# VIS4ROB-lab/ccm_slam

Hardware: AMD Instinct MI355X
Metric: global-BA LM iterations/s (4-agent merged map) (higher is better)
Workload: dtype f64; 1 GPU; gba_c4: global BA (MapFusionGBA numerics), 2000 KFs / 150000 landmarks / 954782 observations, Huber sqrt(5.99), landmark-sharded x1

## Files before the change

### ccm_slam_amd/csrc/ba.hip

```cpp
#include "common.h"
#include "test_internal.h"
#include "ba_types.h"
#include "lane_xor.h"
#include "ba_math.h"
#include <algorithm>
#include <chrono>
#include <cmath>
#include <cstring>
#include <limits>
#include <numeric>

int ccm_allreduce_f64(ccm_ctx* ctx, double* d_buf, size_t n);
int ccm_allreduce_max_f64(ccm_ctx* ctx, double* d_buf, size_t n);

namespace {


inline double now_ms() {
  return std::chrono::duration<double, std::milli>(std::chrono::steady_clock::now().time_since_epoch()).count();
}

__device__ __forceinline__ double wave_sum(double v) { return lanex::wave_sum(v); }

__device__ __forceinline__ double block_sum(double v, double* lds ) {
// ... 1035 lines not shown
    }
    asm volatile("s_waitcnt lgkmcnt(0)" ::: "memory");
  }
  if (el) {
#pragma unroll
    for (int pq = 0; pq < 4; pq++) part[wv][pq][lane] = acc[pq];
  }
  __syncthreads();
  if (threadIdx.x < 4 * 36) {
    const int pq = threadIdx.x / 36, e = threadIdx.x % 36;
    double tot = 0;
#pragma unroll
    for (int k = 0; k < kNW; k++) tot += part[k][pq][e];
    stage_out[((size_t)w * 4 + pq) * 36 + e] = tot;
  }
}

__global__ void ba_coarse_sum(const double* stage, const unsigned* cb_key, int n_cb, int na, int nn, double* Ac, int Nc) {
  const size_t idx = (size_t)blockIdx.x * blockDim.x + threadIdx.x;
  if (idx >= (size_t)Nc * Nc) return;
  const int row = (int)(idx / Nc), col = (int)(idx % Nc);
  if (row >= 6 * nn || col >= 6 * nn) { Ac[idx] = (row == col) ? 1.0 : 0.0; return; }
  int n = row / 6, r = row % 6, n2 = col / 6, c = col % 6;
  if (row > col) { int tmp = n; n = n2; n2 = tmp; tmp = r; r = c; c = tmp; }
  double sum = 0;
#pragma unroll
  for (int pq = 0; pq < 4; pq++) {
    const int p = pq >> 1, q = pq & 1;
    int a = n - p, b = n2 - q;
    if (a < 0 || b < 0 || a >= na || b >= na) continue;
    int sel = 2 * p + q, e = r * 6 + c;
    if (a > b) { const int tmp = a; a = b; b = tmp; sel = 2 * q + p; e = c * 6 + r; }
    const unsigned key = (unsigned)a * (unsigned)na + (unsigned)b;
    int lo = 0, hi = n_cb;
    while (lo < hi) { const int mid = (lo + hi) >> 1; if (cb_key[mid] < key) lo = mid + 1; else hi = mid; }
    if (lo < n_cb && cb_key[lo] == key) sum += stage[((size_t)lo * 4 + sel) * 36 + e];
  }
  Ac[idx] = sum;
}

constexpr long kPersMaxSpins = 8000;
constexpr int kPersCooldownTrials = 8;

struct PersArgs {
  double lambda, rel_tol;
  int max_it, n_clu;
  unsigned* bar;
  int test_abort;
  const int* coff; const int* cij; const uint32_t* cblk;
  unsigned long long* slots;
  unsigned long long* utag;
  unsigned long long* tag;
  int prefetch;
  unsigned long long epoch_base;
  const int* uoff;
  const int* ucol;
  const int* loc;
  long long* dbg;
  const double* Ainv; const double* Pm; int na, Nc;
  double* wsave; int w_load;
};

__device__ __forceinline__ double pers_uniform(double v) {
  const long long b = __double_as_longlong(v);
  const int lo = __builtin_amdgcn_readfirstlane((int)(b & 0xffffffffll)), hi = __builtin_amdgcn_readfirstlane((int)(b >> 32));
  return __longlong_as_double(((long long)hi << 32) | (unsigned int)lo);
}

typedef unsigned int pers_u32x4 __attribute__((ext_vector_type(4)));
constexpr int kAuxSc1 = 16;
__device__ __forceinline__ void tag_store(__amdgpu_buffer_rsrc_t rs, unsigned byte_off, double v, unsigned long long key) {
  const unsigned long long b = (unsigned long long)__double_as_longlong(v), c = b ^ key;
  pers_u32x4 q;
  q.x = (unsigned)b; q.y = (unsigned)(b >> 32); q.z = (unsigned)c; q.w = (unsigned)(c >> 32);
  __builtin_amdgcn_raw_buffer_store_b128(q, rs, (int)byte_off, 0, kAuxSc1);
}
__device__ __forceinline__ pers_u32x4 tag_load(__amdgpu_buffer_rsrc_t rs, unsigned byte_off) { return __builtin_amdgcn_raw_buffer_load_b128(rs, (int)byte_off, 0, kAuxSc1); }
__device__ __forceinline__ bool tag_valid(pers_u32x4 q, unsigned long long key) {
  return (q.x ^ q.z) == (unsigned)key && (q.y ^ q.w) == (unsigned)(key >> 32);
}
__device__ __forceinline__ double tag_value(pers_u32x4 q) { return __longlong_as_double((long long)(((unsigned long long)q.y << 32) | q.x)); }

template <class Mid>
__device__ __forceinline__ bool pers_exchange(int t , unsigned long long* slots , int nwg, int me, double a_thread, double b_thread,
                                              bool force_nan, unsigned long long epoch, unsigned* abort_flag, double* red ,
                                              double* total_a, double* total_b, int* poll_fail ,
                                              Mid&& mid ) {
  const unsigned long long key = 0x9E3779B97F4A7C15ull * epoch;
  {
    const double wa = wave_sum(a_thread), wb = wave_sum(b_thread);
    if ((t & (kWave - 1)) == 0) { red[t / kWave] = wa; red[kPersWaves + t / kWave] = wb; }
  }
  __syncthreads();
  if (t == 0) {
    double ma = 0, mb = 0;
#pragma unroll
    for (int w = 0; w < kPersWaves; w++) { ma += red[w]; mb += red[kPersWaves + w]; }
    if (force_nan) ma = __longlong_as_double(0x7ff8000000000000ll);
    const unsigned long long ba = (unsigned long long)__double_as_longlong(ma), bb = (unsigned long long)__double_as_longlong(mb);
    __hip_atomic_store(slots + me, ba, __ATOMIC_RELAXED, __HIP_MEMORY_SCOPE_AGENT);
    __hip_atomic_store(slots + nwg + me, bb, __ATOMIC_RELAXED, __HIP_MEMORY_SCOPE_AGENT);
    __hip_atomic_store(slots + 2 * nwg + me, ba ^ bb ^ key, __ATOMIC_RELAXED, __HIP_MEMORY_SCOPE_AGENT);
  }
  if (t < kWave) {
    constexpr int kPer = 4;
    unsigned done = 0;
    double va[kPer], vb[kPer];
#pragma unroll
    for (int j = 0; j < kPer; j++) { va[j] = 0; vb[j] = 0; if (t + j * kWave >= nwg) done |= 1u << j; }
    bool ok_w = true;
    for (long spins = 0;; spins++) {
#pragma unroll
      for (int j = 0; j < kPer; j++) {
        if (done & (1u << j)) continue;
        const unsigned long long* in = slots + t + j * kWave;
        const unsigned long long b0 = __hip_atomic_load(in, __ATOMIC_RELAXED, __HIP_MEMORY_SCOPE_AGENT);
        const unsigned long long b1 = __hip_atomic_load(in + nwg, __ATOMIC_RELAXED, __HIP_MEMORY_SCOPE_AGENT);
        const unsigned long long b2 = __hip_atomic_load(in + 2 * nwg, __ATOMIC_RELAXED, __HIP_MEMORY_SCOPE_AGENT);
        if ((b0 ^ b1 ^ b2) == key) { done |= 1u << j; va[j] = __longlong_as_double((long long)b0); vb[j] = __longlong_as_double((long long)b1); }
      }
      if (__all(done == (1u << kPer) - 1u)) break;
      if (spins > kPersMaxSpins || __hip_atomic_load(abort_flag, __ATOMIC_RELAXED, __HIP_MEMORY_SCOPE_AGENT) != 0u) { ok_w = false; break; }
      __builtin_amdgcn_s_sleep(2);
    }
    const double sa = wave_sum(((va[0] + va[1]) + va[2]) + va[3]);
    const double sb = wave_sum(((vb[0] + vb[1]) + vb[2]) + vb[3]);
    if (t == 0) {
      red[2 * kPersWaves] = sa; red[2 * kPersWaves + 1] = sb;
      if (!ok_w) { *poll_fail = 1; __hip_atomic_store(abort_flag, 1u, __ATOMIC_RELAXED, __HIP_MEMORY_SCOPE_AGENT); }
    }
  } else {
    mid();
  }
  __syncthreads();
  const bool alive = *poll_fail == 0;
  *total_a = pers_uniform(red[2 * kPersWaves]);
  *total_b = pers_uniform(red[2 * kPersWaves + 1]);
  return alive;
}

#define PERS_TICK(slot) { if (timing) { const long long tn_ = wall_clock64(); tacc[slot] += tn_ - tacc[12]; tacc[12] = tn_; } }

__device__ __forceinline__ double pers_bcast(double v, int src_lane) {
  const long long b = __double_as_longlong(v);
  const int lo = __builtin_amdgcn_readlane((int)(b & 0xffffffffll), src_lane), hi = __builtin_amdgcn_readlane((int)(b >> 32), src_lane);
  double r = __longlong_as_double(((long long)hi << 32) | (unsigned int)lo);
  asm volatile("" : "+v"(r));
  return r;
}

__device__ __noinline__ void pers_assemble_cluster(double* A, double* Li, const int* cij, const uint32_t* cblk, int c_lo, int c_hi, const double* S, int m,
                                                   double lambda, bool has) {
  constexpr int N = kCluN;
  const int t = threadIdx.x;
  for (int i = t; i < N * N; i += kPersTPB) { A[i] = 0; Li[i] = 0; }
  __syncthreads();
  if (has) {
    const int grp = t / 36, e = t % 36, r = e / 6, cc = e % 6;
    constexpr int kGroups = kPersTPB / 36;
    if (grp < kGroups)
#pragma unroll 4
      for (int s = c_lo + grp; s < c_hi; s += kGroups) {
        const int ij = cij[s], il = ij >> 4, jl = ij & 15;
        const uint32_t bt = cblk[s];
        const double* B = S + 36 * (size_t)(bt & ~kTransposeBit);
        const double v = (bt & kTransposeBit) ? B[cc * 6 + r] : B[e];
        A[(6 * il + r) * N + 6 * jl + cc] = v + ((il == jl && r == cc) ? lambda : 0.0);
      }
  }
  if (m + t < N) A[(m + t) * N + m + t] = 1.0;
  __syncthreads();
}

__device__ __noinline__ void pers_factor_dense(double* A, double* Li, int* ibuf, int m, long long* tacc, bool timing) {
  constexpr int N = kCluN;
  const int t = threadIdx.x;
  PERS_TICK(7)
  double* invd = Li;
  {
    typedef double v4d __attribute__((ext_vector_type(4)));
    const int lane = t & (kWave - 1), wave = __builtin_amdgcn_readfirstlane(t / kWave);
    const int i16 = lane & 15, kq = lane >> 4;
    for (int T = 0; T < 6 && 16 * T < m; T++) {
      const int b0 = 16 * T;
      const int r0 = b0 + 16;
      if (wave < 2) {
        const int rl = lane & 15;
        const int prow = r0 + 48 * wave + (lane - 16);
        const bool is_panel = lane >= 16;
        const int rowi = is_panel ? min(prow, N - 1) : b0 + rl;
        double row[16];
#pragma unroll
        for (int k = 0; k < 16; k++) row[k] = A[rowi * N + b0 + k];
        bool bad = false;
#pragma unroll
        for (int c = 0; c < 16; c++) {
          double sv = row[c];
#pragma unroll
          for (int k = 0; k < c; k++) sv = fma(-row[k], pers_bcast(row[k], c), sv);
          double dd = pers_bcast(sv, c);
          if (!(dd > 0.0)) { bad = true; dd = 1.0; }
          const double inv = rsqrt(dd);
// ... 525 lines not shown
        if (t == c) xres = xc;
      }
      xv[16 * I + t] = xres;
    }
    __syncthreads();
#pragma unroll
    for (int s = 0; s < kCRSlots; s++) {
      const int ij = CR_TIJ(s);
      if ((ij >> 8) == I && (ij & 255) < I) {
        const int J = ij & 255;
        double pv = 0.0;
#pragma unroll
        for (int r = 0; r < 4; r++) pv = fma(acc[s][r], xv[16 * I + kq + 4 * r], pv);
        pv = lanex::add_partner<16>(pv);
        pv = lanex::add_partner<32>(pv);
        if (kq == 0) yv[16 * J + i16] -= pv;
      }
    }
    __syncthreads();
  }
  if (t < n) d.x[t] = xv[t];
  CR_TICK(2)
  {
    double sc = 0;
    if (t < Cp) {
      const int c = d.slot_cam[t];
      double u[6];
#pragma unroll
      for (int q = 0; q < 6; q++) u[q] = xv[6 * t + q];
      const BaPose Tc = ba_load_pose(d.cam[cur] + 7 * (size_t)c);
      const BaPose Tn = ba_oplus(u, Tc);
      ba_store_pose(d.cam[cur ^ 1] + 7 * (size_t)c, Tn);
#pragma unroll
      for (int q = 0; q < 6; q++) sc += u[q] * ((add_lambda_term ? lambda * u[q] : 0.0) + d.bp[6 * (size_t)t + q]);
    }
    if (t < kWave) {
      const double s = wave_sum(sc);
      if (t == 0) d.part_cam[0] = ((s + 0.0) + 0.0) + 0.0;
    }
  }
  CR_TICK(3)
  if (dbg && t == 0) dbg[7] += 1;
#undef CR_TICK
#undef CR_TIJ
  if (t == 0) { d.pcg_flag[0] = 1; d.pcg_flag[1] = 1; d.pcg_flag[2] = ibuf[1]; d.pcg_flag[3] = 0; }
}

__global__ __launch_bounds__(kPersTPB) void ba_pcg_persist(BaDev d, PersArgs a) {
  extern __shared__ __attribute__((aligned(16))) double sm[];
  constexpr int N = kCluN;
  double* A = sm;
  double* Li = sm + N * N;
  double* rc = Li + N * N;
  double* xs = rc + N;
  double* ps = xs + N / 2;
  double* ss = ps + N / 2;
  double* zs = ss + N;
  double* zpart = zs + N;
  double* wl = zpart + 4 * N;
  double* pso = zpart + 8 * N;
  double* red = pso + kPersNcCap;
  int* ibuf = reinterpret_cast<int*>(red + 2 * kPersWaves + 4);
  if (a.test_abort && blockIdx.x == gridDim.x - 1) return;
  const int t = threadIdx.x, lane = t & (kWave - 1);
  const int wv = __builtin_amdgcn_readfirstlane(t / kWave);
  const int nwg = gridDim.x;
  const int per_xcd = nwg >> 3;
  const int u = (blockIdx.x & 7) * per_xcd + (blockIdx.x >> 3);
  const int c = u >> 1, hu = u & 1;
  const bool has = c < a.n_clu;
  const int s0 = has ? c * kClu : 0, s1 = has ? min(d.Cp, s0 + kClu) : 0;
  const int nrows = s1 - s0;
  const int m = 6 * nrows;
  const int o0 = has ? min(s1, s0 + (kClu / 2) * hu) : 0, o1 = has ? min(s1, o0 + kClu / 2) : 0;
  const int nown = o1 - o0;
  const int mo = 6 * nown;
  const int ob = 6 * (o0 - s0);
  unsigned long long epoch = a.epoch_base;
  const double lambda = a.lambda;
  if (t < 4) ibuf[t] = (t == 0) ? 1 : 0;
  long long* tacc = reinterpret_cast<long long*>(ibuf + 4);
  const bool timing = a.dbg != nullptr && blockIdx.x == 0 && t == 0;
  if (timing) { for (int q = 0; q < 12; q++) tacc[q] = 0; tacc[12] = wall_clock64(); }
  if (a.w_load) {
    const double* src = a.wsave + (size_t)u * (N * (N / 2));
    double wreg[5];
    int nw = 0;
    for (int e = t; e < N * (N / 2); e += kPersTPB, nw++) wreg[nw] = src[e];
    nw = 0;
    for (int e = t; e < N * (N / 2); e += kPersTPB, nw++) A[e] = wreg[nw];
    __syncthreads();
  } else {
    pers_factor_cluster(A, Li, ibuf, a.cij, a.cblk, has ? a.coff[c] : 0, has ? a.coff[c + 1] : 0, d.S, s0, s1, lambda, has, tacc, timing);
    double wreg[5];
    int nw = 0;
    for (int e = t; e < N * (N / 2); e += kPersTPB, nw++) wreg[nw] = A[(e / (N / 2)) * N + ob + e % (N / 2)];
    __syncthreads();
    nw = 0;
    double* dst = a.wsave ? a.wsave + (size_t)u * (N * (N / 2)) : nullptr;
    for (int e = t; e < N * (N / 2); e += kPersTPB, nw++) { A[e] = wreg[nw]; if (dst) dst[e] = wreg[nw]; }
  }
  const bool coarse = a.Ainv != nullptr;
  const int Nc = a.Nc, nca = 6 * (a.na + 1);
  float* ainv_l = reinterpret_cast<float*>(A + N * (N / 2));
  double* rco = Li + (32 + 2 * kPersIdxCap + kPersColCap) / 2 + 6 * kPersColCap + 256;
  double* pown = rco + Nc;
  double* ypart = pown + 8 * 36;
  constexpr int kParkA = 8 * N - (4 * N + N / 2);
  double* park_a = zpart + 4 * N + N / 2;
  double* park_b = ypart + 12;
  auto park = [&](int x) { return x < kParkA ? park_a + x : park_b + (x - kParkA); };
  static_assert((32 + 2 * kPersIdxCap + kPersColCap) % 2 == 0 &&
                (32 + 2 * kPersIdxCap + kPersColCap) / 2 + 6 * kPersColCap + 256 + kPersNcCap + 8 * 36 + 12 + (N + kPersNcCap - kParkA) <= kCluN * kCluN,
                "coarse vectors and the parked values do not fit behind the staged structure");
  const int aggu = d.agg >> 3;
  const int agg = u / aggu;
  if (coarse) {
    {
      const double* src = a.Ainv + (size_t)(6 * agg) * Nc;
      double tmpa[9];
#pragma unroll
      for (int q = 0; q < 9; q++) { const int e = t + q * kPersTPB; tmpa[q] = (has && e < 12 * Nc) ? src[e] : 0.0; }
#pragma unroll
      for (int q = 0; q < 9; q++) { const int e = t + q * kPersTPB; if (e < 12 * Nc) ainv_l[e] = (float)tmpa[q]; }
    }
    for (int e = t; e < Nc; e += kPersTPB) { rco[e] = 0.0; pso[e] = 0.0; }
    for (int e = t; e < 8 * 36; e += kPersTPB) pown[e] = (e / 36 < nown) ? a.Pm[36 * (size_t)o0 + e] : 0.0;
  }
  __syncthreads();
  int tq = t, lq = lane;
  auto key_of = [](unsigned long long e) { return 0x9E3779B97F4A7C15ull * e; };
  const unsigned tag_w_pairs = 2u * 6u * (unsigned)d.Cp;
  const __amdgpu_buffer_rsrc_t tag_rs = __builtin_amdgcn_make_buffer_rsrc(a.tag, 0, (int)(16u * (tag_w_pairs + 2u * 8u * (unsigned)kPersNcCap)), 0x00020000);
  auto w_off = [&](unsigned long long e, int i) { return 16u * ((unsigned)(e & 1) * 6u * (unsigned)d.Cp + (unsigned)i); };
  auto c_off = [&](unsigned long long e, int pl, int j) { return 16u * (tag_w_pairs + ((unsigned)(e & 1) * 8u + (unsigned)pl) * (unsigned)kPersNcCap + (unsigned)j); };
  auto coarse_restrict = [&](const double* vec , unsigned long long e ) {
    if (wv == 0) {
      const int cc = lq >> 3, kk = lq & 7;
      double sv = 0;
      if (cc < 6 && kk < nown) {
#pragma unroll
        for (int rr = 0; rr < 6; rr++) sv += pown[kk * 36 + rr * 6 + cc] * vec[6 * kk + rr];
      }
      const double w1 = coarse_hat_t(8 * u + kk, d.agg);
      double s0v = (1.0 - w1) * sv, s1v = w1 * sv;
      s0v = lanex::add_partner<1>(s0v); s1v = lanex::add_partner<1>(s1v);
      s0v = lanex::add_partner<2>(s0v); s1v = lanex::add_partner<2>(s1v);
      s0v = lanex::add_partner<4>(s0v); s1v = lanex::add_partner<4>(s1v);
      if (cc < 6 && kk == 0 && agg < a.na) { tag_store(tag_rs, c_off(e, u - aggu * agg, 6 * agg + cc), s0v, key_of(e)); tag_store(tag_rs, c_off(e, 4 + u - aggu * agg, 6 * (agg + 1) + cc), s1v, key_of(e)); }
    }
  };
  auto fetch_pre = [&](unsigned long long e, bool want_w) {
    const unsigned long long key = key_of(e);
    int tf = tq;
    asm volatile("" : "+v"(tf));
    const int p = tf - kWave, j = p - N;
    const bool is_w = want_w && p >= 0 && p < m && !(p >= ob && p < ob + mo);
    const bool is_c = coarse && j >= 0 && j < nca;
    const int n = j / 6;
    bool ok = true;
    double sgm = 0;
    for (int h = 0; h < 2 && 2 * h < aggu; h++) {
      unsigned off[2] = {c_off(e, 2 * h, j), c_off(e, 4 + 2 * h, j)}, want = 0;
#pragma unroll
      for (int i = 0; i < 4; i++) {
        const int mm = 2 * h + (i >> 1);
        const bool first = (i & 1) == 0;
        const int unit = first ? aggu * n + mm : aggu * (n - 1) + mm;
        if (is_c && mm < aggu && (first ? n < a.na : n >= 1) && unit < nwg) want |= 1u << i;
      }
      if (is_w) { want = (h == 0) ? 1u : 0u; off[0] = w_off(e, 6 * s0 + p); }
      unsigned todo = want;
      pers_u32x4 q[4];
#pragma unroll
      for (int i = 0; i < 4; i++) q[i] = pers_u32x4{0u, 0u, 0u, 0u};
      for (int spins = 0; todo; spins++) {
        asm volatile("" ::: "memory");
#pragma unroll
        for (int i = 0; i < 4; i++) if (todo & (1u << i)) q[i] = tag_load(tag_rs, off[i & 1] + 16u * (unsigned)kPersNcCap * (unsigned)(i >> 1));
#pragma unroll
        for (int i = 0; i < 4; i++) if ((todo & (1u << i)) && tag_valid(q[i], key)) todo &= ~(1u << i);
        if (!todo) break;
        if (spins > kPersMaxSpins || __hip_atomic_load(a.bar + 1, __ATOMIC_RELAXED, __HIP_MEMORY_SCOPE_AGENT) != 0u) { ok = false; break; }
        __builtin_amdgcn_s_sleep(1);
      }
      if (is_w) { if (h == 0) *park(p) = tag_value(q[0]); }
      else {
#pragma unroll
        for (int i = 0; i < 4; i++) if (want & (1u << i)) sgm += tag_value(q[i]);
      }
      if (!ok) break;
    }
    if (is_c) *park(p) = sgm;
    if (!ok) { ibuf[2] = 1; __hip_atomic_store(a.bar + 1, 1u, __ATOMIC_RELAXED, __HIP_MEMORY_SCOPE_AGENT); }
  };
  if (t < N / 2) { xs[t] = 0; ps[t] = 0; }
  if (t < N) { ss[t] = 0; zs[t] = 0; rc[t] = (t < m) ? d.bs[6 * (size_t)s0 + t] : 0.0; }
  __syncthreads();
  PERS_TICK(10)
  int* l_off = reinterpret_cast<int*>(Li);
  int* l_loc = l_off + 32;
  uint32_t* l_blk = reinterpret_cast<uint32_t*>(l_loc + kPersIdxCap);
  int* l_ucol = reinterpret_cast<int*>(l_blk + kPersIdxCap);
  double* pl = reinterpret_cast<double*>(l_ucol + kPersColCap);
  double* half_sum = pl + 6 * kPersColCap;
  const int e_base = has ? d.row_off[o0] : 0;
  const int n_ent = has ? d.row_off[o1] - e_base : 0;
  const int u_base = has ? a.uoff[u] : 0;
  const int nu = has ? a.uoff[u + 1] - u_base : 0;
  if (has) {
    if (t <= nown) l_off[t] = d.row_off[o0 + t] - e_base;
    for (int s = t; s < n_ent; s += kPersTPB) { l_loc[s] = a.loc[e_base + s]; l_blk[s] = d.row_blk[e_base + s]; }
    for (int s = t; s < nu; s += kPersTPB) l_ucol[s] = a.ucol[u_base + s];
  }
  if (t < 6) pl[t] = 0.0;
  __syncthreads();
  constexpr int kPersRegEnt = 5;
  const int row_l = wv >> 1, half = wv & 1, g = lane / 6, r = lane % 6;
  const bool row_ok = has && row_l < nown && g < 10;
  double sreg[kPersRegEnt][6];
  int jreg[kPersRegEnt];
  {
    const int e0 = row_ok ? l_off[row_l] : 0;
    const int e_end = row_ok ? l_off[row_l + 1] : 0;
#pragma unroll
    for (int k = 0; k < kPersRegEnt; k++) {
      const int s = e0 + half * 10 + g + 20 * k;
      const bool v = row_ok && s < e_end;
      jreg[k] = v ? 6 * l_loc[s] : 0;
      const uint32_t bt = v ? l_blk[s] : 0u;
      const double* B = d.S + 36 * (size_t)(bt & ~kTransposeBit);
#pragma unroll
      for (int q = 0; q < 6; q++) sreg[k][q] = v ? ((bt & kTransposeBit) ? B[q * 6 + r] : B[r * 6 + q]) : 0.0;
    }
  }
  auto apply_W = [&](unsigned long long ukey) {
    {
      const int row = tq % (N / 2), prt = tq / (N / 2);
      if (prt < 8) {
        double sv = 0;
        if (row < mo) {
          const int c0 = prt * 12;
#pragma unroll
          for (int col = 0; col < 12; col++) sv += A[(c0 + col) * (N / 2) + row] * rc[c0 + col];
        }
        zpart[prt * (N / 2) + row] = sv;
      } else if (coarse && wv < 12) {
        const float* ar0 = ainv_l + (wv - 6) * Nc;
        const float* ar1 = ainv_l + (wv - 6 + 6) * Nc;
        double acc0 = 0, acc1 = 0;
        for (int j = lq; j < nca; j += kWave) { const double rv = rco[j]; acc0 += (double)ar0[j] * rv; acc1 += (double)ar1[j] * rv; }
        acc0 = wave_sum(acc0); acc1 = wave_sum(acc1);
        if (lq == 0) { ypart[wv - 6] = acc0; ypart[wv - 6 + 6] = acc1; }
      }
    }
    __syncthreads();
    double rz = 0;
    if (tq < mo) {
      double z = zpart[tq];
#pragma unroll
      for (int q = 1; q < 8; q++) z += zpart[q * (N / 2) + tq];
      if (coarse) {
        const int kk = tq / 6, rr = tq % 6;
        const double w1 = coarse_hat_t(8 * u + kk, d.agg), w0 = 1.0 - w1;
#pragma unroll
        for (int cc = 0; cc < 6; cc++) z += pown[kk * 36 + rr * 6 + cc] * (w0 * ypart[cc] + w1 * ypart[6 + cc]);
      }
      zs[tq] = z;
      const unsigned long long zb = (unsigned long long)__double_as_longlong(z);
      unsigned long long* dst = a.utag + 2 * (6 * (size_t)o0 + tq);
      __hip_atomic_store(dst, zb, __ATOMIC_RELAXED, __HIP_MEMORY_SCOPE_AGENT);
      __hip_atomic_store(dst + 1, zb ^ ukey, __ATOMIC_RELAXED, __HIP_MEMORY_SCOPE_AGENT);
      rz = rc[ob + tq] * z;
    }
    return rz;
  };
  auto halo_load = [&](unsigned long long ukey) {
    constexpr int kPer = (6 * kPersColCap + kPersTPB - 1) / kPersTPB;
    unsigned done = 0;
#pragma unroll
    for (int i = 0; i < kPer; i++) if (tq + i * kPersTPB >= 6 * nu) done |= 1u << i;
    bool ok = true;
    for (long spins = 0; done != (1u << kPer) - 1u; spins++) {
#pragma unroll
      for (int i = 0; i < kPer; i++) {
        if (done & (1u << i)) continue;
        const int idx = tq + i * kPersTPB;
        const unsigned long long* src = a.utag + 2 * (6 * (size_t)l_ucol[idx / 6] + idx % 6);
        const unsigned long long b0 = __hip_atomic_load(src, __ATOMIC_RELAXED, __HIP_MEMORY_SCOPE_AGENT);
        const unsigned long long b1 = __hip_atomic_load(src + 1, __ATOMIC_RELAXED, __HIP_MEMORY_SCOPE_AGENT);
        if ((b0 ^ b1) == ukey) { done |= 1u << i; pl[idx] = __longlong_as_double((long long)b0); }
      }
      if (done == (1u << kPer) - 1u) break;
      if (spins > kPersMaxSpins || __hip_atomic_load(a.bar + 1, __ATOMIC_RELAXED, __HIP_MEMORY_SCOPE_AGENT) != 0u) { ok = false; break; }
      __builtin_amdgcn_s_sleep(1);
    }
    if (!ok) { ibuf[2] = 1; __hip_atomic_store(a.bar + 1, 1u, __ATOMIC_RELAXED, __HIP_MEMORY_SCOPE_AGENT); }
    __syncthreads();
    return ibuf[2] == 0;
  };
  auto spmv_w = [&](unsigned long long e , double* wu) {
    double acc = 0;
#pragma unroll
    for (int kk = 0; kk < kPersRegEnt; kk++) {
      int jo = jreg[kk];
      asm volatile("" : "+v"(jo), "+v"(acc));
      const double* pj = pl + jo;
#pragma unroll
      for (int q = 0; q < 6; q++) acc += sreg[kk][q] * pj[q];
    }
    {
      const int gq = lq / 6, rq = lq - 6 * gq;
      const bool rowq = has && row_l < nown && gq < 10;
      const int e_endq = rowq ? l_off[row_l + 1] : 0;
      for (int s = (rowq ? l_off[row_l] : 0) + half * 10 + gq + 20 * kPersRegEnt; s < e_endq; s += 20) {
        const uint32_t bt = l_blk[s];
        const double* B = d.S + 36 * (size_t)(bt & ~kTransposeBit);
        const double* pj = pl + 6 * l_loc[s];
#pragma unroll
        for (int q = 0; q < 6; q++) acc += ((bt & kTransposeBit) ? B[q * 6 + rq] : B[rq * 6 + q]) * pj[q];
      }
    }
    acc += __shfl_down(acc, 30, kWave);
    const double pr = acc + __shfl_down(acc, 6, kWave);
    acc = (pr + __shfl_down(pr, 12, kWave)) + __shfl_down(acc, 24, kWave);
    if (lq < 6) half_sum[(row_l * 2 + half) * 8 + lq] = acc;
    __syncthreads();
    double wu_t = 0;
    if (tq < mo) {
      const int rw = tq / 6, cc = tq % 6;
      const double ui = zs[tq];
      const double wv_ = (half_sum[(rw * 2) * 8 + cc] + half_sum[(rw * 2 + 1) * 8 + cc]) + lambda * ui;
      wl[tq] = wv_;
      tag_store(tag_rs, w_off(e, 6 * o0 + tq), wv_, key_of(e));
      wu_t = wv_ * ui;
    }
    *wu = wu_t;
  };
  auto slots_of = [&](unsigned long long e) { return a.slots + 3 * (size_t)nwg * (e & 1); };
  auto exchange = [&](unsigned long long e, double a_t, double b_t, bool force_nan, double* ta, double* tb, bool want_w) {
    const bool ok = pers_exchange(tq, slots_of(e), nwg, u, a_t, b_t, force_nan, e, a.bar + 1, red, ta, tb, ibuf + 2, [&]() { if (a.prefetch) fetch_pre(e, want_w); });
    if (!a.prefetch && tq >= kWave) fetch_pre(e, want_w);
    return ok;
  };
  int fail = 0, k = 0;
  double gam = 0, del = 0;
  bool alive = true;
  if (coarse) {
    coarse_restrict(rc + ob, epoch + 1);
    double dummy = 0, dummy2 = 0;
    alive = exchange(epoch + 1, 0.0, 0.0, false, &dummy, &dummy2, false);
    ++epoch;
    if (t >= kWave + N && t - (kWave + N) < nca) rco[t - (kWave + N)] += *park(t - kWave);
    __syncthreads();
  }
  if (alive) {
    const double ru_t = apply_W(key_of(epoch + 1));
    alive = halo_load(key_of(epoch + 1));
    double wu_t = 0;
    spmv_w(epoch + 1, &wu_t);
    if (coarse) { __syncthreads(); coarse_restrict(wl, epoch + 1); }
    const bool alive2 = exchange(epoch + 1, ru_t, wu_t, has && ibuf[1], &gam, &del, true);
    ++epoch;
    alive = alive && alive2;
  }
  const double gam0 = gam;
  const double thresh = a.rel_tol * a.rel_tol;
  double gam_prev = gam, alpha_prev = 1.0;
  if (!alive) fail = 1;
  PERS_TICK(11)
  for (; alive && k < a.max_it; k++) {
    tq = t; asm volatile("" : "+v"(tq)); lq = tq & (kWave - 1);
    if (gam <= thresh * gam0 || !(gam > 0.0)) { if (gam != gam) fail = 1; break; }
    const double beta = pers_uniform((k == 0) ? 0.0 : gam / gam_prev);
    const double pap = (k == 0) ? del : del - beta * gam / alpha_prev;
    if (!(pap > 0.0)) { fail = 1; break; }
    const double alpha = pers_uniform(gam / pap);
    {
      const int p = tq - kWave, j = p - N;
      if (tq < mo) { const double pi = zs[tq] + beta * ps[tq]; ps[tq] = pi; xs[tq] += alpha * pi; }
      if (p >= 0 && p < m) { const double si = ((p >= ob && p < ob + mo) ? wl[p - ob] : *park(p)) + beta * ss[p]; ss[p] = si; rc[p] -= alpha * si; }
      if (coarse && j >= 0 && j < nca) { const double sc = *park(p) + beta * pso[j]; pso[j] = sc; rco[j] -= alpha * sc; }
    }
    __syncthreads();
    PERS_TICK(0)
    const double ru_t = apply_W(key_of(epoch + 1));
    PERS_TICK(1)
    long long tw0 = 0;
    if (a.dbg && t == 0) tw0 = wall_clock64();
    alive = halo_load(key_of(epoch + 1));
    if (a.dbg && t == 0) a.dbg[33 + 2 * u] += wall_clock64() - tw0;
    PERS_TICK(2)
    if (!alive) { fail = 1; break; }
    double wu_t = 0;
    spmv_w(epoch + 1, &wu_t);
    if (coarse) { __syncthreads(); coarse_restrict(wl, epoch + 1); }
    PERS_TICK(3)
    gam_prev = gam; alpha_prev = alpha;
    if (a.dbg && t == 0) tw0 = wall_clock64();
    alive = exchange(epoch + 1, ru_t, wu_t, false, &gam, &del, true);
    ++epoch;
    if (a.dbg && t == 0) a.dbg[32 + 2 * u] += wall_clock64() - tw0;
    PERS_TICK(4)
    if (!alive) { fail = 1; break; }
  }
#undef PERS_TICK
  if (timing) { for (int q = 0; q < 12; q++) a.dbg[q] += tacc[q]; a.dbg[12] += k; a.dbg[13] += 1; }
  if (t < mo) d.x[6 * (size_t)o0 + t] = xs[t];
  if (blockIdx.x == 0 && t == 0) {
    d.pcg_flag[0] = 1; d.pcg_flag[1] = k; d.pcg_flag[2] = fail;
    d.pcg_flag[3] = ibuf[2] | (int)__hip_atomic_load(a.bar + 1, __ATOMIC_RELAXED, __HIP_MEMORY_SCOPE_AGENT);
  }
}

__global__ __launch_bounds__(kPersTPB) void ba_pcg_init_tiles(BaDev d, double lambda, double rel_tol, const int* coff, const int* cij, const uint32_t* cblk) {
  extern __shared__ __attribute__((aligned(16))) double sm[];
  constexpr int N = kCluN;
  double* A = sm;
  double* Li = sm + N * N;
  double* rc = Li + N * N;
  double* red = rc + N;
  int* ibuf = reinterpret_cast<int*>(red + kPersWaves);
  const int t = threadIdx.x, c = blockIdx.x;
  const int s0 = c * kClu, s1 = min(d.Cp, s0 + kClu);
  const int m = 6 * (s1 - s0);
  if (t < 4) ibuf[t] = 0;
  __syncthreads();
  pers_factor_cluster(A, Li, ibuf, cij, cblk, coff[c], coff[c + 1], d.S, s0, s1, lambda, true, nullptr, false);
  float* W = d.Wc + (size_t)c * N * N;
  for (int e = t; e < N * N; e += kPersTPB) W[e] = (float)A[e];
  if (t < N) rc[t] = (t < m) ? d.bs[6 * (size_t)s0 + t] : 0.0;
  __syncthreads();
  double rz = 0;
  if (t < m) {
    double z = 0;
    for (int col = 0; col < m; col++) z += (double)(float)A[col * N + t] * rc[col];
    const size_t g = 6 * (size_t)s0 + t;
    d.x[g] = 0; d.r[g] = rc[t]; d.z[g] = z; d.p[0][g] = 0;
    rz = rc[t] * z;
  }
  rz = wave_sum(rz);
  if ((t & (kWave - 1)) == 0) red[t / kWave] = rz;
  __syncthreads();
  if (t == 0) {
    double tot = 0;
    for (int w = 0; w < kPersWaves; w++) tot += red[w];
    d.prz[0][c] = tot;
    d.prz[1][c] = 0;
    if (ibuf[1]) d.pcg_flag[2] = 1;
    if (c == 0) { d.pcg_scal[1] = rel_tol * rel_tol; d.pcg_scal[2] = lambda; }
  }
  if (d.mk_on) mk_restrict(d, c, s0, m, rc, Li);
}

constexpr size_t kPersLdsBytes = (size_t)(2 * kCluN * kCluN + 4 * kCluN + 8 * kCluN + kPersNcCap + 2 * kPersWaves + 4) * sizeof(double) + 16 + 14 * sizeof(long long);
static_assert(kPersLdsBytes <= 160 * 1024, "persistent PCG: LDS of one workgroup exceeds the 160 KB of a CU");
static inline size_t pers_lds_bytes() { return kPersLdsBytes; }

static PersArgs pers_args(ccm_ba* ba, double lambda, double rel_tol, int max_it) {
  PersArgs pa{};
  pa.lambda = lambda; pa.rel_tol = rel_tol; pa.max_it = max_it; pa.n_clu = ccm_div_up(ba->d.Cp, kClu);
  pa.bar = ba->d_pers_bar; pa.slots = (unsigned long long*)ba->d_pers_part;
  pa.utag = (unsigned long long*)ba->d_pers_u; pa.tag = ba->d_pers_tag; pa.prefetch = ba->pers_prefetch ? 1 : 0;
  pa.epoch_base = (++ba->pers_launch) << 20;
  pa.uoff = ba->d_pers_uoff; pa.ucol = ba->d_pers_ucol; pa.loc = ba->d_pers_loc;
  pa.coff = ba->d_pers_coff; pa.cij = ba->d_pers_cij; pa.cblk = ba->d_pers_cblk;
  return pa;
}
static void pers_args_coarse(const ccm_ba* ba, PersArgs* pa) { pa->Ainv = ba->d_cAinv; pa->Pm = ba->d_cP; pa->na = ba->coarse_na; pa->Nc = ba->coarse_Nc; }


template <int TPB>
__device__ __forceinline__ double block_dot_small(double v, double* red ) {
  v = wave_sum(v);
  if (TPB == kWave) return v;
  __syncthreads();
  if ((threadIdx.x & (kWave - 1)) == 0) red[threadIdx.x / kWave] = v;
  __syncthreads();
  double s = 0;
#pragma unroll
  for (int i = 0; i < TPB / kWave; i++) s += red[i];
  return s;
}
// ... 1120 lines not shown
```

### ccm_slam_amd/csrc/ba_build.hip

```cpp
#include "common.h"
#include "ba_types.h"
#include "ba_math.h"
#include "ba_sort.h"
#include <algorithm>
#include <chrono>
#include <cstring>
#include <rocprim/rocprim.hpp>

int ccm_ba_build_pairs(ccm_ctx* ctx, const int* d_pt_off, const int* d_cslot, int Lp, int Cp, int lb, int le, int eb,
                       uint32_t** d_U_out, int* nOff_out, int** d_inst_off, int** d_inst_a, int** d_inst_c, int64_t* n_inst,
                       std::vector<std::pair<void*, size_t>>& keep);
int ccm_ba_pers_grid_fits(ccm_ctx* ctx, int grid);
int ccm_ba_state_from_raw(ccm_ba* ba);

namespace {

constexpr int kB = 256;

inline double now_ms() { return std::chrono::duration<double, std::milli>(std::chrono::steady_clock::now().time_since_epoch()).count(); }

struct BuildSizes {
  int Cp, Lp, Eact, bad, max_cam_edges, n_fix_edges, worst_units, n_units, pers_bad, n_ucol, n_cij, ncb, pad[4];
};

// ... 679 lines not shown
      const size_t nk = (size_t)Cp + nOff;
      unsigned* ck = nullptr; int* cv = nullptr;
      BB_RC(tmp.get(nk, &ck)); BB_RC(tmp.get(nk, &cv)); BB_RC(tmp.get(nk, &uq)); BB_RC(tmp.get(nk + 1, &cnts)); BB_RC(tmp.get(1, &n_runs));
      hipLaunchKernelGGL(bb_coarse_keys, dim3(grid_for((int64_t)nk)), dim3(kB), 0, st, Cp, nOff, (const int*)ba->d_blk_i, (const int*)ba->d_blk_j, na, agg, ck, cv);
      unsigned* ck_s = ck; int* cv_s = cv;
      BB_RC(sort_pairs(ctx, tmp, ck, cv, nk, bits_for((uint64_t)na * na), &ck_s, &cv_s));
      BB_RC(keep_get(ba, nk, &ba->d_cb_ent));
      BB_HIP(hipMemcpyAsync(ba->d_cb_ent, cv_s, nk * sizeof(int), hipMemcpyDeviceToDevice, st));
      size_t bytes = 0;
      BB_HIP(rocprim::run_length_encode(nullptr, bytes, ck_s, (unsigned)nk, uq, cnts, n_runs, st));
      char* scratch = nullptr;
      BB_RC(tmp.get(bytes, &scratch));
      BB_HIP(rocprim::run_length_encode(scratch, bytes, ck_s, (unsigned)nk, uq, cnts, n_runs, st));
      const size_t max_runs = std::min<size_t>(nk, (size_t)na * (na + 1) / 2);
      BB_RC(keep_get(ba, max_runs + 1, &ba->d_cb_off)); BB_RC(keep_get(ba, 2 * max_runs, &ba->d_cb_ab));
      BB_RC(keep_get(ba, max_runs, &ba->d_cb_key)); BB_RC(keep_get(ba, max_runs * 4 * 36, &ba->d_cstage));
      BB_HIP(hipMemcpyAsync(ba->d_cb_key, uq, max_runs * sizeof(unsigned), hipMemcpyDeviceToDevice, st));
      hipLaunchKernelGGL(bb_counts_tail, dim3(1), dim3(1), 0, st, cnts, (const int*)n_runs);
      BB_RC(scan_excl(ctx, tmp, (const int*)cnts, ba->d_cb_off, max_runs + 1));
      hipLaunchKernelGGL(bb_coarse_ab, dim3(grid_for((int64_t)max_runs)), dim3(kB), 0, st, (const unsigned*)uq, (const int*)n_runs, na, ba->d_cb_ab, sz);
    }
    BB_HIP(hipGetLastError());
    BB_HIP(hipMemcpyAsync(&hs, sz, sizeof(hs), hipMemcpyDeviceToHost, st));
    BB_HIP(hipStreamSynchronize(st));
    lap("rows, lists, unit offsets");
    d.max_cam_edges = hs.max_cam_edges;
    d.unit_tab = nullptr; d.row_unit_off = nullptr; d.blk_unit0 = nullptr; d.row_units_max = 0; d.row_dbg = nullptr;
    if (ccm_dbg("row")) { long long* p_dbg = nullptr; BB_RC(keep_get(ba, 8, &p_dbg, true)); d.row_dbg = p_dbg; }
    if (nOff > row_min_blocks() && d.max_cam_edges <= kRowMaxEdges && (uint64_t)std::max(Eloc, 1) * 144u < (1ull << 31)) {
      const size_t lds_free = 158 * 1024 - ((size_t)(d.max_cam_edges + 1) * 18 + 27 * (size_t)ccm_div_up(d.max_cam_edges, kRow2Group)) * sizeof(double);
      const int units_cap = (int)(lds_free / (36 * sizeof(double)));
      if (hs.worst_units <= units_cap) {
        int4* p_tab = nullptr;
        BB_RC(keep_get(ba, (size_t)hs.n_units, &p_tab));
        hipLaunchKernelGGL(bb_unit_fill, dim3(Cp), dim3(kB), 3 * (size_t)std::max(hs.worst_units, 1) * sizeof(int), st, Cp, unit_chunk, (const int*)p_rowblk,
                           (const int*)d_inst_off, (const int*)p_row_u, (const int*)p_blk_u, p_tab);
        BB_HIP(hipGetLastError());
        d.unit_tab = p_tab; d.row_unit_off = p_row_u; d.blk_unit0 = p_blk_u; d.row_units_max = std::max(hs.worst_units, 1);
      }
    }
#define AL(field, n, T) { T* _p = nullptr; BB_RC(keep_get<T>(ba, (n), &_p, true)); d.field = _p; }
    AL(cam[0], 7 * (size_t)n_cam, double) AL(cam[1], 7 * (size_t)n_cam, double)
    AL(pt[0], 3 * (size_t)Lloc, double) AL(pt[1], 3 * (size_t)Lloc, double)
    d.E4L = nullptr;
    d.w_free = (d.E4 && d.chunk_off && d.unit_tab && nOff > row_min_blocks()) ? 1 : 0;
    if (d.w_free) { double* p_l = nullptr; BB_RC(keep_get(ba, 4 * (size_t)Eloc, &p_l)); d.E4L = p_l; }
    AL(W, d.w_free ? 1 : 18 * (size_t)Eloc, double) AL(Hll, 6 * (size_t)Lloc, double) AL(bl, 3 * (size_t)Lloc, double)
    AL(Dinv, 6 * (size_t)Lloc, double) AL(dl, 3 * (size_t)Lloc, double) AL(Hpp, 36 * (size_t)Cp, double) AL(bp, 6 * (size_t)Cp, double)
    AL(x, 6 * (size_t)Cp, double) AL(r, 6 * (size_t)Cp, double) AL(z, 6 * (size_t)Cp, double) AL(q, 6 * (size_t)Cp, double)
    AL(p[0], 6 * (size_t)Cp, double) AL(p[1], 6 * (size_t)Cp, double)
    AL(Wc, (size_t)n_cl * kCluN * kCluN, float)
    d.n_wg_spmv = ((ccm_div_up(std::max(Cp, 1), kRowsPerWG) + 7) / 8) * 8;
    d.n_wg_wave4 = ccm_div_up(std::max(Cp, 1), kTPB / kWave);
    d.n_wg_upd = n_cl;
    d.n_wg_pt = ccm_div_up(std::max(Lloc, 1), kTPB); d.n_wg_cam = ccm_div_up(std::max(Cp, 1), kTPB);
    d.n_part = d.chunk_off ? d.n_chunk : d.n_wg_pt;
    AL(ppq, d.n_wg_spmv, double) AL(prz[0], d.n_wg_upd, double) AL(prz[1], d.n_wg_upd, double)
    AL(pcg_scal, 4, double)
    AL(edge_chi2, Eloc, double) AL(edge_depth, Eloc, uint8_t)
    AL(part_pt, 2 * (size_t)std::max(d.n_wg_pt, d.n_chunk), double) AL(part_cam, d.n_wg_cam, double) AL(scal, 8, double)
#undef AL
    d.pcg_flag = reinterpret_cast<int*>(d.scal + 6);
    if (!ctx->rb_free.empty()) { ba->h_rb = static_cast<double*>(ctx->rb_free.back()); ctx->rb_free.pop_back(); }
    else if (hipHostMalloc(&ba->h_rb, 128, hipHostMallocCoherent ) != hipSuccess) return ccm_set_error(ctx, CCM_E_HIP, "ccm_ba_create: pinned read-back buffer");
    memset(ba->h_rb, 0, 128);
    ba->red_count = 36 * (size_t)(Cp + nOff) + 6 * (size_t)Cp;
    BB_RC(keep_get(ba, ba->red_count, &ba->d_red, true));
    d.S = ba->d_red; d.bs = ba->d_red + 36 * (size_t)(Cp + nOff);
    BB_RC(keep_get(ba, 3 * (size_t)std::max(Lp, 1), &ba->d_pt_full, true));
    BB_RC(keep_get(ba, 36 * (size_t)std::max(Cp, 1), &ba->d_hpp_full, true));
    auto coarse_buffers = [&]() -> int {
      BB_RC(keep_get(ba, 36 * (size_t)Cp, &ba->d_cP, true));
      BB_RC(keep_get(ba, (size_t)Nc * Nc, &ba->d_cA, true)); BB_RC(keep_get(ba, (size_t)Nc * Nc, &ba->d_cX, true));
      BB_RC(keep_get(ba, (size_t)Nc * Nc, &ba->d_cAinv, true)); BB_RC(keep_get(ba, (size_t)Nc * 64, &ba->d_cLinv, true));
      BB_RC(keep_get(ba, 4, &ba->d_cinfo, true));
      ba->coarse_na = na; ba->coarse_Nc = Nc; ba->coarse_ncb = hs.ncb;
      if (const char* cf = getenv("CCM_BA_COARSE")) ba->coarse_force = !strcmp(cf, "always") ? 1 : !strcmp(cf, "never") ? -1 : 0;
      return CCM_OK;
    };
    ba->pers_grid = 0;
    d.mk_cpart = nullptr; d.mk_cry[0] = d.mk_cry[1] = nullptr; d.mk_P = nullptr; d.mk_Ainv = nullptr; d.mk_Ainv32 = nullptr; d.mk_on = 0; d.mk_Nc = 0; d.mk_na = 0;
    if (pers_try && !hs.pers_bad) {
      BB_RC(keep_get(ba, 4 + 2 * 16 + 4 * 512, &ba->d_pers_bar, true));
      BB_RC(keep_get(ba, 6 * (size_t)pers_grid_want, &ba->d_pers_part, true));
      BB_RC(keep_get(ba, 12 * (size_t)Cp, &ba->d_pers_u, true));
      BB_RC(keep_get(ba, 2 * (2 * 6 * (size_t)Cp + 2 * 8 * (size_t)kPersNcCap), &ba->d_pers_tag, true));
      { const char* pf = getenv("CCM_BA_PERS_PREFETCH"); ba->pers_prefetch = !(pf && !strcmp(pf, "0")); }
      ba->pers_grid = pers_grid_want; ba->pers_grid_built = pers_grid_want;
      BB_RC(keep_get(ba, (size_t)pers_grid_want * (kCluN * (kCluN / 2)), &ba->d_pers_wsave, false));
      if (coarse_pers) BB_RC(coarse_buffers());
    } else if (pers_try) { ba->d_pers_uoff = nullptr; ba->d_pers_ucol = nullptr; ba->d_pers_loc = nullptr; }
    if (Cp > kSmallMaxCp && Cp <= kDense2MaxCp && ba->d_pers_coff)
      BB_RC(keep_get(ba, (size_t)kCluN * kCluN + 16, &ba->d_dense_T, true));
    if (cholreg_win) {
      const size_t np = 16 * (size_t)ccm_div_up(6 * Cp, 16);
      BB_RC(keep_get(ba, 16, &ba->d_cholreg_dbg, true));
      BB_RC(keep_get(ba, np * np, &ba->d_cholreg_L, false));
      BB_RC(keep_get(ba, (size_t)8 * 24 * 64 * 4, &ba->d_cholreg_tab, false));
    }
    if (!ba->pers_grid && coarse_mk) {
      BB_RC(coarse_buffers());
      double *p1 = nullptr, *p2 = nullptr, *p3 = nullptr;
      BB_RC(keep_get(ba, 24 * (size_t)(na + 1), &p1, true)); BB_RC(keep_get(ba, (size_t)n_cl, &p2, true)); BB_RC(keep_get(ba, (size_t)n_cl, &p3, true));
      d.mk_cpart = p1; d.mk_cry[0] = p2; d.mk_cry[1] = p3;
      d.mk_P = ba->d_cP; d.mk_Ainv = ba->d_cAinv; d.mk_Nc = Nc; d.mk_na = na;
      BB_RC(keep_get(ba, (size_t)Nc * Nc, &ba->d_cAinv32, false)); d.mk_Ainv32 = ba->d_cAinv32;
    }
    d.S32 = nullptr; d.qx = nullptr;
    if (!ba->pers_grid && pers_wanted && pers_grid_want > 4 * kWave) {
      float* p32 = nullptr;
      BB_RC(keep_get(ba, 36 * (size_t)(Cp + nOff), &p32, false));
      d.S32 = p32;
      double* pqx = nullptr;
      BB_RC(keep_get(ba, 6 * (size_t)Cp, &pqx, false));
      d.qx = pqx;
    }
    BB_RC(flush_zero_list(ba));
    BB_RC(ccm_ba_state_from_raw(ba));
    BB_HIP(hipStreamSynchronize(st));
    lap("unit table, buffers, state");
    return CCM_OK;
  };
  rc_build = body();
  }
  if (rc_build != CCM_OK) { ccm_ba_destroy(ba); return rc_build; }
  ba->ms_setup = now_ms() - t0;
  *out = ba;
  return CCM_OK;
}
```

Baseline: 975.2 LM iter/s.

## Use packed buffer-load tags for exchange slots and drop initial coarse exchange

Cross-workgroup reduction slots and the utag halo now use 128-bit raw buffer stores and loads with a sc1 cache policy, replacing separate 64-bit atomic stores and loads. This cuts the number of memory transactions per poll. The initial coarse restriction moves before the factorization and reads Pm directly, so the extra grid-wide exchange before the CG loop can be replaced by a local fetch. This relies on the restriction tags being published early enough, and the slot buffer grows from 6 to 8 words per workgroup.

```diff
diff --git a/ccm_slam_amd/csrc/ba.hip b/ccm_slam_amd/csrc/ba.hip
--- a/ccm_slam_amd/csrc/ba.hip
+++ b/ccm_slam_amd/csrc/ba.hip
@@ -1141,7 +1141,8 @@
 __device__ __forceinline__ double tag_value(pers_u32x4 q) { return __longlong_as_double((long long)(((unsigned long long)q.y << 32) | q.x)); }
 
 template <class Mid>
-__device__ __forceinline__ bool pers_exchange(int t , unsigned long long* slots , int nwg, int me, double a_thread, double b_thread,
+__device__ __forceinline__ bool pers_exchange(int t , __amdgpu_buffer_rsrc_t slot_rs , unsigned set_off ,
+                                              int nwg, int me, double a_thread, double b_thread,
                                               bool force_nan, unsigned long long epoch, unsigned* abort_flag, double* red ,
                                               double* total_a, double* total_b, int* poll_fail ,
                                               Mid&& mid ) {
@@ -1157,9 +1158,12 @@
     for (int w = 0; w < kPersWaves; w++) { ma += red[w]; mb += red[kPersWaves + w]; }
     if (force_nan) ma = __longlong_as_double(0x7ff8000000000000ll);
     const unsigned long long ba = (unsigned long long)__double_as_longlong(ma), bb = (unsigned long long)__double_as_longlong(mb);
-    __hip_atomic_store(slots + me, ba, __ATOMIC_RELAXED, __HIP_MEMORY_SCOPE_AGENT);
-    __hip_atomic_store(slots + nwg + me, bb, __ATOMIC_RELAXED, __HIP_MEMORY_SCOPE_AGENT);
-    __hip_atomic_store(slots + 2 * nwg + me, ba ^ bb ^ key, __ATOMIC_RELAXED, __HIP_MEMORY_SCOPE_AGENT);
+    const unsigned long long bc = ba ^ bb ^ key;
+    pers_u32x4 q0, q1;
+    q0.x = (unsigned)ba; q0.y = (unsigned)(ba >> 32); q0.z = (unsigned)bb; q0.w = (unsigned)(bb >> 32);
+    q1.x = (unsigned)bc; q1.y = (unsigned)(bc >> 32); q1.z = 0u; q1.w = 0u;
+    __builtin_amdgcn_raw_buffer_store_b128(q0, slot_rs, (int)(set_off + 32u * (unsigned)me), 0, kAuxSc1);
+    __builtin_amdgcn_raw_buffer_store_b128(q1, slot_rs, (int)(set_off + 32u * (unsigned)me + 16u), 0, kAuxSc1);
   }
   if (t < kWave) {
     constexpr int kPer = 4;
@@ -1169,14 +1173,17 @@
     for (int j = 0; j < kPer; j++) { va[j] = 0; vb[j] = 0; if (t + j * kWave >= nwg) done |= 1u << j; }
     bool ok_w = true;
     for (long spins = 0;; spins++) {
+      asm volatile("" ::: "memory");
 #pragma unroll
       for (int j = 0; j < kPer; j++) {
         if (done & (1u << j)) continue;
-        const unsigned long long* in = slots + t + j * kWave;
-        const unsigned long long b0 = __hip_atomic_load(in, __ATOMIC_RELAXED, __HIP_MEMORY_SCOPE_AGENT);
-        const unsigned long long b1 = __hip_atomic_load(in + nwg, __ATOMIC_RELAXED, __HIP_MEMORY_SCOPE_AGENT);
-        const unsigned long long b2 = __hip_atomic_load(in + 2 * nwg, __ATOMIC_RELAXED, __HIP_MEMORY_SCOPE_AGENT);
-        if ((b0 ^ b1 ^ b2) == key) { done |= 1u << j; va[j] = __longlong_as_double((long long)b0); vb[j] = __longlong_as_double((long long)b1); }
+        const unsigned in = set_off + 32u * (unsigned)(t + j * kWave);
+        const pers_u32x4 q0 = tag_load(slot_rs, in), q1 = tag_load(slot_rs, in + 16u);
+        if ((q0.x ^ q0.z ^ q1.x) == (unsigned)key && (q0.y ^ q0.w ^ q1.y) == (unsigned)(key >> 32)) {
+          done |= 1u << j;
+          va[j] = __longlong_as_double((long long)(((unsigned long long)q0.y << 32) | q0.x));
+          vb[j] = __longlong_as_double((long long)(((unsigned long long)q0.w << 32) | q0.z));
+        }
       }
       if (__all(done == (1u << kPer) - 1u)) break;
       if (spins > kPersMaxSpins || __hip_atomic_load(abort_flag, __ATOMIC_RELAXED, __HIP_MEMORY_SCOPE_AGENT) != 0u) { ok_w = false; break; }
@@ -1868,6 +1875,34 @@
   long long* tacc = reinterpret_cast<long long*>(ibuf + 4);
   const bool timing = a.dbg != nullptr && blockIdx.x == 0 && t == 0;
   if (timing) { for (int q = 0; q < 12; q++) tacc[q] = 0; tacc[12] = wall_clock64(); }
+  int tq = t, lq = lane;
+  const bool coarse = a.Ainv != nullptr;
+  const int aggu = d.agg >> 3;
+  const int agg = u / aggu;
+  auto key_of = [](unsigned long long e) { return 0x9E3779B97F4A7C15ull * e; };
+  const unsigned tag_w_pairs = 2u * 6u * (unsigned)d.Cp;
+  const __amdgpu_buffer_rsrc_t tag_rs = __builtin_amdgcn_make_buffer_rsrc(a.tag, 0, (int)(16u * (tag_w_pairs + 2u * 8u * (unsigned)kPersNcCap)), 0x00020000);
+  const __amdgpu_buffer_rsrc_t u_rs = __builtin_amdgcn_make_buffer_rsrc(a.utag, 0, (int)(16u * 6u * (unsigned)d.Cp), 0x00020000);
+  const __amdgpu_buffer_rsrc_t slot_rs = __builtin_amdgcn_make_buffer_rsrc(a.slots, 0, (int)(2u * 32u * (unsigned)nwg), 0x00020000);
+  auto w_off = [&](unsigned long long e, int i) { return 16u * ((unsigned)(e & 1) * 6u * (unsigned)d.Cp + (unsigned)i); };
+  auto c_off = [&](unsigned long long e, int pl, int j) { return 16u * (tag_w_pairs + ((unsigned)(e & 1) * 8u + (unsigned)pl) * (unsigned)kPersNcCap + (unsigned)j); };
+  auto coarse_restrict = [&](const double* pk , const double* vec , unsigned long long e ) {
+    if (wv == 0) {
+      const int cc = lq >> 3, kk = lq & 7;
+      double sv = 0;
+      if (cc < 6 && kk < nown) {
+#pragma unroll
+        for (int rr = 0; rr < 6; rr++) sv += pk[kk * 36 + rr * 6 + cc] * vec[6 * kk + rr];
+      }
+      const double w1 = coarse_hat_t(8 * u + kk, d.agg);
+      double s0v = (1.0 - w1) * sv, s1v = w1 * sv;
+      s0v = lanex::add_partner<1>(s0v); s1v = lanex::add_partner<1>(s1v);
+      s0v = lanex::add_partner<2>(s0v); s1v = lanex::add_partner<2>(s1v);
+      s0v = lanex::add_partner<4>(s0v); s1v = lanex::add_partner<4>(s1v);
+      if (cc < 6 && kk == 0 && agg < a.na) { tag_store(tag_rs, c_off(e, u - aggu * agg, 6 * agg + cc), s0v, key_of(e)); tag_store(tag_rs, c_off(e, 4 + u - aggu * agg, 6 * (agg + 1) + cc), s1v, key_of(e)); }
+    }
+  };
+  if (coarse) coarse_restrict(a.Pm + 36 * (size_t)o0, d.bs + 6 * (size_t)o0, epoch + 1);
   if (a.w_load) {
     const double* src = a.wsave + (size_t)u * (N * (N / 2));
     double wreg[5];
@@ -1886,7 +1921,6 @@
     double* dst = a.wsave ? a.wsave + (size_t)u * (N * (N / 2)) : nullptr;
     for (int e = t; e < N * (N / 2); e += kPersTPB, nw++) { A[e] = wreg[nw]; if (dst) dst[e] = wreg[nw]; }
   }
-  const bool coarse = a.Ainv != nullptr;
   const int Nc = a.Nc, nca = 6 * (a.na + 1);
   float* ainv_l = reinterpret_cast<float*>(A + N * (N / 2));
   double* rco = Li + (32 + 2 * kPersIdxCap + kPersColCap) / 2 + 6 * kPersColCap + 256;
@@ -1899,8 +1933,6 @@
   static_assert((32 + 2 * kPersIdxCap + kPersColCap) % 2 == 0 &&
                 (32 + 2 * kPersIdxCap + kPersColCap) / 2 + 6 * kPersColCap + 256 + kPersNcCap + 8 * 36 + 12 + (N + kPersNcCap - kParkA) <= kCluN * kCluN,
                 "coarse vectors and the parked values do not fit behind the staged structure");
-  const int aggu = d.agg >> 3;
-  const int agg = u / aggu;
   if (coarse) {
     {
       const double* src = a.Ainv + (size_t)(6 * agg) * Nc;
@@ -1914,28 +1946,6 @@
     for (int e = t; e < 8 * 36; e += kPersTPB) pown[e] = (e / 36 < nown) ? a.Pm[36 * (size_t)o0 + e] : 0.0;
   }
   __syncthreads();
-  int tq = t, lq = lane;
-  auto key_of = [](unsigned long long e) { return 0x9E3779B97F4A7C15ull * e; };
-  const unsigned tag_w_pairs = 2u * 6u * (unsigned)d.Cp;
-  const __amdgpu_buffer_rsrc_t tag_rs = __builtin_amdgcn_make_buffer_rsrc(a.tag, 0, (int)(16u * (tag_w_pairs + 2u * 8u * (unsigned)kPersNcCap)), 0x00020000);
-  auto w_off = [&](unsigned long long e, int i) { return 16u * ((unsigned)(e & 1) * 6u * (unsigned)d.Cp + (unsigned)i); };
-  auto c_off = [&](unsigned long long e, int pl, int j) { return 16u * (tag_w_pairs + ((unsigned)(e & 1) * 8u + (unsigned)pl) * (unsigned)kPersNcCap + (unsigned)j); };
-  auto coarse_restrict = [&](const double* vec , unsigned long long e ) {
-    if (wv == 0) {
-      const int cc = lq >> 3, kk = lq & 7;
-      double sv = 0;
-      if (cc < 6 && kk < nown) {
-#pragma unroll
-        for (int rr = 0; rr < 6; rr++) sv += pown[kk * 36 + rr * 6 + cc] * vec[6 * kk + rr];
-      }
-      const double w1 = coarse_hat_t(8 * u + kk, d.agg);
-      double s0v = (1.0 - w1) * sv, s1v = w1 * sv;
-      s0v = lanex::add_partner<1>(s0v); s1v = lanex::add_partner<1>(s1v);
-      s0v = lanex::add_partner<2>(s0v); s1v = lanex::add_partner<2>(s1v);
-      s0v = lanex::add_partner<4>(s0v); s1v = lanex::add_partner<4>(s1v);
-      if (cc < 6 && kk == 0 && agg < a.na) { tag_store(tag_rs, c_off(e, u - aggu * agg, 6 * agg + cc), s0v, key_of(e)); tag_store(tag_rs, c_off(e, 4 + u - aggu * agg, 6 * (agg + 1) + cc), s1v, key_of(e)); }
-    }
-  };
   auto fetch_pre = [&](unsigned long long e, bool want_w) {
     const unsigned long long key = key_of(e);
     int tf = tq;
@@ -2053,10 +2063,7 @@
         for (int cc = 0; cc < 6; cc++) z += pown[kk * 36 + rr * 6 + cc] * (w0 * ypart[cc] + w1 * ypart[6 + cc]);
       }
       zs[tq] = z;
-      const unsigned long long zb = (unsigned long long)__double_as_longlong(z);
-      unsigned long long* dst = a.utag + 2 * (6 * (size_t)o0 + tq);
-      __hip_atomic_store(dst, zb, __ATOMIC_RELAXED, __HIP_MEMORY_SCOPE_AGENT);
-      __hip_atomic_store(dst + 1, zb ^ ukey, __ATOMIC_RELAXED, __HIP_MEMORY_SCOPE_AGENT);
+      tag_store(u_rs, 16u * (unsigned)(6 * o0 + tq), z, ukey);
       rz = rc[ob + tq] * z;
     }
     return rz;
@@ -2068,14 +2075,13 @@
     for (int i = 0; i < kPer; i++) if (tq + i * kPersTPB >= 6 * nu) done |= 1u << i;
     bool ok = true;
     for (long spins = 0; done != (1u << kPer) - 1u; spins++) {
+      asm volatile("" ::: "memory");
 #pragma unroll
       for (int i = 0; i < kPer; i++) {
         if (done & (1u << i)) continue;
         const int idx = tq + i * kPersTPB;
-        const unsigned long long* src = a.utag + 2 * (6 * (size_t)l_ucol[idx / 6] + idx % 6);
-        const unsigned long long b0 = __hip_atomic_load(src, __ATOMIC_RELAXED, __HIP_MEMORY_SCOPE_AGENT);
-        const unsigned long long b1 = __hip_atomic_load(src + 1, __ATOMIC_RELAXED, __HIP_MEMORY_SCOPE_AGENT);
-        if ((b0 ^ b1) == ukey) { done |= 1u << i; pl[idx] = __longlong_as_double((long long)b0); }
+        const pers_u32x4 q = tag_load(u_rs, 16u * (unsigned)(6 * l_ucol[idx / 6] + idx % 6));
+        if (tag_valid(q, ukey)) { done |= 1u << i; pl[idx] = tag_value(q); }
       }
       if (done == (1u << kPer) - 1u) break;
       if (spins > kPersMaxSpins || __hip_atomic_load(a.bar + 1, __ATOMIC_RELAXED, __HIP_MEMORY_SCOPE_AGENT) != 0u) { ok = false; break; }
@@ -2123,20 +2129,19 @@
     }
     *wu = wu_t;
   };
-  auto slots_of = [&](unsigned long long e) { return a.slots + 3 * (size_t)nwg * (e & 1); };
-  auto exchange = [&](unsigned long long e, double a_t, double b_t, bool force_nan, double* ta, double* tb, bool want_w) {
-    const bool ok = pers_exchange(tq, slots_of(e), nwg, u, a_t, b_t, force_nan, e, a.bar + 1, red, ta, tb, ibuf + 2, [&]() { if (a.prefetch) fetch_pre(e, want_w); });
-    if (!a.prefetch && tq >= kWave) fetch_pre(e, want_w);
+  auto exchange = [&](unsigned long long e, double a_t, double b_t, bool force_nan, double* ta, double* tb) {
+    const bool ok = pers_exchange(tq, slot_rs, 32u * (unsigned)nwg * (unsigned)(e & 1), nwg, u, a_t, b_t, force_nan, e, a.bar + 1, red, ta, tb, ibuf + 2, [&]() { if (a.prefetch) fetch_pre(e, true); });
+    if (!a.prefetch && tq >= kWave) fetch_pre(e, true);
     return ok;
   };
   int fail = 0, k = 0;
   double gam = 0, del = 0;
   bool alive = true;
   if (coarse) {
-    coarse_restrict(rc + ob, epoch + 1);
-    double dummy = 0, dummy2 = 0;
-    alive = exchange(epoch + 1, 0.0, 0.0, false, &dummy, &dummy2, false);
+    if (t >= kWave) fetch_pre(epoch + 1, false);
     ++epoch;
+    __syncthreads();
+    alive = ibuf[2] == 0;
     if (t >= kWave + N && t - (kWave + N) < nca) rco[t - (kWave + N)] += *park(t - kWave);
     __syncthreads();
   }
@@ -2145,8 +2150,8 @@
     alive = halo_load(key_of(epoch + 1));
     double wu_t = 0;
     spmv_w(epoch + 1, &wu_t);
-    if (coarse) { __syncthreads(); coarse_restrict(wl, epoch + 1); }
-    const bool alive2 = exchange(epoch + 1, ru_t, wu_t, has && ibuf[1], &gam, &del, true);
+    if (coarse) { __syncthreads(); coarse_restrict(pown, wl, epoch + 1); }
+    const bool alive2 = exchange(epoch + 1, ru_t, wu_t, has && ibuf[1], &gam, &del);
     ++epoch;
     alive = alive && alive2;
   }
@@ -2180,11 +2185,11 @@
     if (!alive) { fail = 1; break; }
     double wu_t = 0;
     spmv_w(epoch + 1, &wu_t);
-    if (coarse) { __syncthreads(); coarse_restrict(wl, epoch + 1); }
+    if (coarse) { __syncthreads(); coarse_restrict(pown, wl, epoch + 1); }
     PERS_TICK(3)
     gam_prev = gam; alpha_prev = alpha;
     if (a.dbg && t == 0) tw0 = wall_clock64();
-    alive = exchange(epoch + 1, ru_t, wu_t, false, &gam, &del, true);
+    alive = exchange(epoch + 1, ru_t, wu_t, false, &gam, &del);
     ++epoch;
     if (a.dbg && t == 0) a.dbg[32 + 2 * u] += wall_clock64() - tw0;
     PERS_TICK(4)
diff --git a/ccm_slam_amd/csrc/ba_build.hip b/ccm_slam_amd/csrc/ba_build.hip
--- a/ccm_slam_amd/csrc/ba_build.hip
+++ b/ccm_slam_amd/csrc/ba_build.hip
@@ -785,7 +785,7 @@
     d.mk_cpart = nullptr; d.mk_cry[0] = d.mk_cry[1] = nullptr; d.mk_P = nullptr; d.mk_Ainv = nullptr; d.mk_Ainv32 = nullptr; d.mk_on = 0; d.mk_Nc = 0; d.mk_na = 0;
     if (pers_try && !hs.pers_bad) {
       BB_RC(keep_get(ba, 4 + 2 * 16 + 4 * 512, &ba->d_pers_bar, true));
-      BB_RC(keep_get(ba, 6 * (size_t)pers_grid_want, &ba->d_pers_part, true));
+      BB_RC(keep_get(ba, 8 * (size_t)pers_grid_want, &ba->d_pers_part, true));
       BB_RC(keep_get(ba, 12 * (size_t)Cp, &ba->d_pers_u, true));
       BB_RC(keep_get(ba, 2 * (2 * 6 * (size_t)Cp + 2 * 8 * (size_t)kPersNcCap), &ba->d_pers_tag, true));
       { const char* pf = getenv("CCM_BA_PERS_PREFETCH"); ba->pers_prefetch = !(pf && !strcmp(pf, "0")); }
```

New measurement: 1010 LM iter/s, median of 6. 3.6% higher.
